# pglira/simpleICP

Measured on AMD Instinct MI355X. Metric: ICP iterations/sec (kNN correspondences/sec in `correspondences_per_s`), 10M-vs-10M pts, higher is better.
Workload: dtype f64; 1 GPU; C4 synthetic 10000000-vs-10000000 surface (SURVEY 8d generator), correspondences=1000, neighbors=10, exact 1-NN (bit-identical to brute force); n_fixed=10000000, n_movable=10000000, correspondences=1000, neighbors=10, parallelism=movable-cloud index shards x1, queries replicated

## Files before the change

simpleicp_amd/_lib.py:

```python
from __future__ import annotations

import ctypes as C
import os
from pathlib import Path

import numpy as np

PKG = Path(__file__).resolve().parent
LIB_PATH = Path(os.environ["SICP_LIBRARY"]) if os.environ.get("SICP_LIBRARY") else PKG / "libsimpleicp_hip.so"

FIX, MOV = 0, 1
OK, ERR_INVALID, ERR_HIP, ERR_NO_DEVICE, ERR_TOO_FEW, ERR_NUMERIC, ERR_EXCHANGE = 0, -1, -2, -3, -4, -5, -6
XCHG_ALLGATHER_F64, XCHG_SUM_F64, XCHG_MIN_U64, XCHG_MAX_U64 = 1, 2, 3, 4
PART_CLOUD, PART_QUERIES = 0, 1
K_KNN1, K_KNNK, K_NORMALEQ, K_SELECT, K_XCHG = 0, 1, 2, 3, 4
ABI_VERSION = 7
KERNEL_NAMES = {K_KNN1: "match", K_KNNK: "knnk_scan", K_NORMALEQ: "solve", K_SELECT: "reject_select", K_XCHG: "exchange"}
MATCH_KERNELS = {0: "k_knn1_scan", 1: "k_knn1_fscan", 2: "k_grid_nn", 3: "k_knn1_frec", 5: "k_grid_nn16", 6: "k_grid_nn16f"}

EXPORTS = [
    "sicp_abi_version", "sicp_last_error", "sicp_device_count", "sicp_ctx_create", "sicp_ctx_destroy",
    "sicp_ctx_device_name", "sicp_cloud_upload", "sicp_cloud_upload_columns", "sicp_cloud_upload_start", "sicp_cloud_upload_wait", "sicp_cloud_size", "sicp_cloud_transform",
    "sicp_cloud_download", "sicp_cloud_download_columns", "sicp_cloud_download_both", "sicp_cloud_set_planarity", "sicp_knn", "sicp_select_in_range", "sicp_estimate_normals", "sicp_icp_setup", "sicp_icp_iterate",
    "sicp_icp_run", "sicp_icp_get_state", "sicp_icp_uncertainties", "sicp_icp_normal_equations", "sicp_params_to_H",
# ... 5 lines not shown
BATCH_EXPORTS = ["sicp_batch_version", "sicp_icp_run_batch", "sicp_ctx_lean"]
BATCH_VERSION = 1
BATCH_PATH_BATCHED, BATCH_PATH_FALLBACK = 1, 2

DEVICE_EXPORTS = ["sicp_device_version", "sicp_cloud_upload_strided", "sicp_select_n_device", "sicp_select_positions",
                  "sicp_cloud_write_strided"]
DEVICE_VERSION = 1
DT_F32, DT_F64 = 1, 2

NORMALS_EXPORTS = ["sicp_normals_version", "sicp_cloud_set_normals", "sicp_normal_angle_set", "sicp_corr_reject_normal_angle",
                   "sicp_normal_angle_info", "sicp_normal_cache_read"]
NORMALS_VERSION = 1

VOXEL_EXPORTS = ["sicp_voxel_version", "sicp_voxel_select", "sicp_voxel_select_masked"]
VOXEL_VERSION = 1


class BackendError(RuntimeError):

    def __init__(self, message, code=None):
        super().__init__(message)
        self.code = code


class IterParams(C.Structure):
    _fields_ = [("x", C.c_double * 6), ("obs", C.c_double * 6), ("obs_weight", C.c_double * 6),
                ("min_planarity", C.c_double), ("distance_weight", C.c_double), ("max_lm_steps", C.c_int64)]


class IterResult(C.Structure):
# ... 104 lines not shown
        for name in DEVICE_EXPORTS:
            getattr(L, name).restype = cint
    if all(hasattr(L, name) for name in NORMALS_EXPORTS):
        L.sicp_cloud_set_normals.argtypes = [vp, cint, vp, vp, i64, i64]
        L.sicp_normal_angle_set.argtypes = [vp, dbl, cint]
        L.sicp_corr_reject_normal_angle.argtypes = [vp, dbl, cint, vp, vp, C.POINTER(i64)]
        L.sicp_normal_angle_info.argtypes = [vp, vp]
        L.sicp_normal_cache_read.argtypes = [vp, vp, vp]
        for name in NORMALS_EXPORTS:
            getattr(L, name).restype = cint
    if all(hasattr(L, name) for name in VOXEL_EXPORTS):
        L.sicp_voxel_select.argtypes = [vp, cint, vp, i64, dbl, vp, vp, C.POINTER(i64)]
        L.sicp_voxel_select_masked.argtypes = [vp, cint, vp, i64, dbl, vp, vp, C.POINTER(i64)]
        for name in VOXEL_EXPORTS:
            getattr(L, name).restype = cint
    _lib = L
    return L


def _ptr(a):
    if a is None:
        return None
    if isinstance(a, np.ndarray):
        return a.ctypes.data_as(C.c_void_p)
    if hasattr(a, "data_ptr"):
        return C.c_void_p(a.data_ptr())
    raise TypeError(f"unsupported buffer type {type(a)}")


def _f64(a):
# ... 543 lines not shown
        self._chk(self._L.sicp_match_work(self._h, _ptr(out)))
        d = C.c_uint64(0)
        self._chk(self._L.sicp_match_deferred(self._h, C.byref(d)))
        return {"candidates": int(out[0]), "rows": int(out[1]), "launches": int(out[2]), "deferred": int(d.value)}

    def tail_cycles(self):
        out = np.zeros(5)
        self._chk(self._L.sicp_tail_cycles(self._h, _ptr(out)))
        return dict(zip(("load", "select", "keep", "lm", "final"), (float(v) for v in out)))

    def tail_selection(self):
        out = np.zeros(3, np.int64)
        self._chk(self._L.sicp_tail_selection(self._h, _ptr(out)))
        return {"median_rounds": int(out[0]), "mad_rounds": int(out[1]), "window_iterations": int(out[2])}

    def exchange_info(self):
        out = np.zeros(4, np.int64)
        self._chk(self._L.sicp_exchange_info(self._h, _ptr(out)))
        return {"form": ("none", "records_allgather", "key_allreduces", "query_slices")[int(out[0])], "count": int(out[1]),
                "keys_min_q": int(out[2]), "callback_serves_u64": bool(out[3])}

    def knn_work(self):
        out = np.zeros(4, np.uint64)
        self._chk(self._L.sicp_knn_work(self._h, _ptr(out)))
        return {"candidates": int(out[0]), "sweeps": int(out[1]), "slow_queries": int(out[2]), "in_ball": int(out[3])}

    def timing(self):
        out = {}
        for k, name in KERNEL_NAMES.items():
            ms, n = C.c_double(), C.c_int64()
# ... 4 lines not shown
```

simpleicp_amd/build.py:

```python
import os
import shutil
import subprocess
import sys
from concurrent.futures import ThreadPoolExecutor
from pathlib import Path

PKG = Path(__file__).resolve().parent
CSRC = PKG / "csrc"
LIB = PKG / "libsimpleicp_hip.so"
SOURCES = [CSRC / "sicp_api.cpp", CSRC / "sicp_clouds.cpp", CSRC / "sicp_search.cpp", CSRC / "sicp_icp.cpp", CSRC / "sicp_comm.cpp", CSRC / "sicp_kernels.hip", CSRC / "sicp_grid.hip", CSRC / "sicp_gridf.hip", CSRC / "sicp_tail.hip", CSRC / "sicp_reject.hip", CSRC / "sicp_lm.hip", CSRC / "sicp_batch.hip", CSRC / "sicp_device.hip", CSRC / "sicp_nangle.hip", CSRC / "sicp_voxel.hip", CSRC / "sicp_io.cpp"]
HEADERS = [CSRC / "sicp_internal.h", CSRC / "sicp_host.h", CSRC / "sicp_lanes.h", CSRC / "sicp_solver.h", CSRC / "sicp_normals.h", CSRC / "sicp_grid_dev.h",
           CSRC / "sicp_grid_nn_one.inc", CSRC / "sicp_knn_sweep4.inc", CSRC / "sicp_tail_body.inc", PKG.parent / "include" / "simpleicp_hip.h",
           PKG.parent / "include" / "simpleicp_hip_batch.h", PKG.parent / "include" / "simpleicp_hip_device.h",
           PKG.parent / "include" / "simpleicp_hip_normals.h", PKG.parent / "include" / "simpleicp_hip_voxel.h"]
COMPILE = ["--offload-arch=gfx950", "-O3", "-std=c++17", "-ffp-contract=off", "-fPIC",
           "-fvisibility=hidden", "-Wall", "-pthread", "-mllvm", "-amdgpu-mfma-vgpr-form",
           "-mllvm", "-amdgpu-kernarg-preload-count=16"]
LINK = ["--offload-arch=gfx950", "-shared", "-fPIC", "-pthread"]
OBJ = PKG / "_obj"
LIB_ASAN = OBJ / "libsimpleicp_hip_asan.so"


def hipcc():
    exe = shutil.which("hipcc") or "/opt/rocm/bin/hipcc"
    if not Path(exe).exists():
        raise RuntimeError("hipcc not found: cannot build libsimpleicp_hip.so")
    return exe


# ... 79 lines not shown
```

simpleicp_amd/csrc/sicp_api.cpp:

```cpp
#include "sicp_host.h"

namespace sicph {

thread_local std::string g_err;

int fail(int code, const char *fmt, ...)
{
    char buf[512];
    va_list ap;
    va_start(ap, fmt);
    vsnprintf(buf, sizeof buf, fmt, ap);
    va_end(ap);
    g_err = buf;
    return code;
}

}

int sicp_io_fail(int code, const char *fmt, ...)
{
    char buf[512];
    va_list ap;
    va_start(ap, fmt);
    vsnprintf(buf, sizeof buf, fmt, ap);
// ... 120 lines not shown
    if (rc == SICP_OK && hipMemsetAsync(c->ticket.p, 0, 4 * sizeof(unsigned), c->stream) != hipSuccess) rc = SICP_ERR_HIP;
    if (rc != SICP_OK) { sicp_ctx_destroy(c); return rc; }
    if (const char *e = std::getenv("SICP_ORDER_MIN_Q")) c->order_min_q = std::atol(e);
    if (const char *e = std::getenv("SICP_KNN_SWEEP")) c->knn_sweep = std::atoi(e) != 0;
    if (const char *e = std::getenv("SICP_KNN_BATCH")) c->knn_batch = std::atol(e);
    if (const char *e = std::getenv("SICP_KNN_GROUP")) c->knn_group = std::atoi(e);
    if (const char *e = std::getenv("SICP_NN16_MIN_Q")) c->nn16_min_q = std::atol(e);
    if (const char *e = std::getenv("SICP_NN16")) c->nn16_filter = !std::strcmp(e, "exact") ? 0 : !std::strcmp(e, "far") ? 1 : 2;
    if (const char *e = std::getenv("SICP_BOXES")) { c->use_boxes = std::atoi(e) != 0; c->boxes_always = std::atoi(e) >= 2; }
    if (const char *e = std::getenv("SICP_NN16F_MIN_Q")) { c->nn16f_min_q = std::atol(e); c->nn16f_min_q_forced = true; }
    if (const char *e = std::getenv("SICP_FAR_MOVE")) { const double t = std::atof(e); if (t >= 0) c->far_move = t; }
    if (const char *e = std::getenv("SICP_COARSE_MIN_N")) c->coarse_min_n = std::atol(e);
    if (const char *e = std::getenv("SICP_LM")) c->lm_one_launch = std::strcmp(e, "launches") != 0;
    if (const char *e = std::getenv("SICP_HSEL_WINDOW")) c->hsel_window = std::atoi(e) != 0;
    if (const char *e = std::getenv("SICP_TAIL_WINDOW")) c->tail_window = std::atoi(e) != 0;
    if (const char *e = std::getenv("SICP_TEST_BARRIER_FAULT")) c->test_barrier_fault = std::atoi(e);
    if (const char *e = std::getenv("SICP_NN_GROUP")) { const int v = std::atoi(e); if (v == 8 || v == 16) c->nn_group = v; }
    if (const char *e = std::getenv("SICP_XCHG_KEYS_MIN_Q")) c->xkeys_min_q = std::atol(e);
    if (const char *e = std::getenv("SICP_COMM_TIMEOUT_S")) { const double v = std::atof(e); if (v > 0) c->xchg_timeout_s = 2.0 * v; }
    if (const char *e = std::getenv("SICP_FSCAN")) c->fscan_variant = !std::strcmp(e, "inline") ? 1 : 0;
    if (const char *e = std::getenv("SICP_FSCAN_CAP")) c->fscan_cap = std::atol(e);
    if (const char *e = std::getenv("SICP_SOLVE_TRACE")) {
        c->solve_trace = true;
        c->host_trace = std::strstr(e, "host") != nullptr;
        c->trace_sel = std::strstr(e, "sel") != nullptr; c->trace_eval = std::strstr(e, "eval") != nullptr;
    }
    if (const char *e = std::getenv("SICP_SOLVE")) c->solve_mode = !std::strcmp(e, "fused") ? 1 : !std::strcmp(e, "host") ? 2 : 0;
    if (const char *e = std::getenv("SICP_KNN1"))
        c->knn1_mode = !std::strcmp(e, "exact") ? 1 : !std::strcmp(e, "filter") ? 2 : !std::strcmp(e, "grid") ? 3 : 0;
    *ctx_out = c;
// ... 91 lines not shown
    HIPCHK(hipMemcpyAsync(out, c->match_work.p + 3, sizeof(uint64_t), hipMemcpyDeviceToHost, c->stream));
    return sync(c);
}
SICP_EXPORT int sicp_tail_cycles(sicp_ctx *c, double out5[5])
{
    if (!c || !out5) return fail(SICP_ERR_INVALID, "null argument");
    std::memcpy(out5, c->last_tail_cycles, sizeof c->last_tail_cycles);
    return SICP_OK;
}
SICP_EXPORT int sicp_tail_selection(sicp_ctx *c, int64_t out3[3])
{
    if (!c || !out3) return fail(SICP_ERR_INVALID, "null argument");
    out3[0] = c->last_sel_rounds[0]; out3[1] = c->last_sel_rounds[1]; out3[2] = c->sel_window_hits;
    return SICP_OK;
}
SICP_EXPORT int sicp_knn_work(sicp_ctx *c, uint64_t out4[4])
{
    if (!c || !out4) return fail(SICP_ERR_INVALID, "null argument");
    HIPCHK(hipSetDevice(c->device));
    HIPCHK(hipMemcpyAsync(out4, c->match_work.p + 4, 4 * sizeof(uint64_t), hipMemcpyDeviceToHost, c->stream));
    return sync(c);
}
SICP_EXPORT int sicp_timing_reset(sicp_ctx *c)
{
    if (!c) return fail(SICP_ERR_INVALID, "null ctx");
    if (!c->pending.empty()) CHK(sync(c));
    HIPCHK(hipMemsetAsync(c->match_work.p, 0, 8 * sizeof(unsigned long long), c->stream));
    for (int i = 0; i < SICP_K_COUNT; ++i) { c->t_ms[i] = 0; c->t_n[i] = 0; }
    return SICP_OK;
}
// ... 10 lines not shown
```

simpleicp_amd/csrc/sicp_batch.hip:

```cpp
#include "sicp_host.h"
#include "../../include/simpleicp_hip_batch.h"

#include <set>

namespace {

void set_status(sicp_batch_member &m, int rc)
{
    m.status = rc;
    if (rc == SICP_OK) m.error[0] = '\0';
    else std::snprintf(m.error, sizeof m.error, "%s", sicp_last_error());
}

bool batchable(sicp_ctx *c, const sicp_batch_member &m)
{
    if (check_iter_args(c, &m.params) != SICP_OK) return false;
    if (!device_tail(c) || c->Q > SOLVE_MAX_Q || !takes_grid_search(c)) return false;
    if (normal_angle_on(c)) return false;
    return !(c->timing || c->count_work || c->host_trace || c->solve_trace);
}

struct MemberRun {
    int64_t idx;
    double xcur[6];
// ... 82 lines not shown
        run.push_back(r);
    }
    const long B = (long)tab.size();
    if (B > 0) {
        std::vector<uint32_t> map;
        int depth = 1 << 30;
        int64_t max_all = 0;
        for (long k = 0; k < B; ++k) {
            const long blocks = ((long)tab[k].A.Q + 3) / 4;
            tab[k].blk0 = (uint32_t)map.size();
            map.insert(map.end(), (size_t)blocks, (uint32_t)k);
            depth = std::min(depth, mem[run[k].idx].ctx->chain_depth);
            max_all = std::max(max_all, tab[k].max_it);
        }
        const long nblk = (long)map.size();
        const int epts[4] = {1, 2, 4, 8};
        long b_off[4], b_cnt[4];
        for (int b = 0; b < 4; ++b) {
            b_off[b] = (long)map.size();
            for (long k = 0; k < B; ++k)
                if (icp_tail_ept(tab[k].A.Q) == epts[b]) map.push_back((uint32_t)k);
            b_cnt[b] = (long)map.size() - b_off[b];
        }
        for (long k = 0; k < B; ++k) tab[k].ring = c0->h_batch_ring + (size_t)k * REC_RING * REC_DOUBLES;
        const hipStream_t s0 = c0->stream;
        const int rc = [&]() -> int {
        for (long k = 0; k < B; ++k) HIPCHK(hipStreamWaitEvent(s0, mem[run[k].idx].ctx->batch_ev, 0));
        HIPCHK(hipMemcpyAsync(c0->batch_tab.p, tab.data(), (size_t)B * sizeof(BatchMember), hipMemcpyHostToDevice, s0));
        HIPCHK(hipMemcpyAsync(c0->batch_map.p, map.data(), map.size() * sizeof(uint32_t), hipMemcpyHostToDevice, s0));
        for (long k = 0; k < B; ++k) {
            sicp_ctx *c = mem[run[k].idx].ctx;
            c->have_prev_match = true;
            c->last_match_kernel = 2;
        }

        double seqs[REC_RING];
        int64_t launched = 0, completed = 0;
        auto all_over = [&]() {
            for (long k = 0; k < B; ++k) if (!run[k].over && launched < tab[k].max_it) return false;
            return true;
        };
        while (true) {
            while (launched < max_all && launched - completed < depth && !all_over()) {
                const double seq = (double)(++c0->solve_seq);
                const int slot = (int)(launched % REC_RING);
                seqs[slot] = seq;
                launch_grid_nn_batch(s0, c0->batch_tab.p, c0->batch_map.p, nblk, launched);
                for (int b = 0; b < 4; ++b)
                    if (b_cnt[b] > 0) launch_icp_tail_batch(s0, epts[b], c0->batch_tab.p, c0->batch_map.p + b_off[b], b_cnt[b], launched, slot, seq);
                HIPCHK(hipGetLastError());
                ++launched;
            }
            if (completed == launched) break;
            const int slot = (int)(completed % REC_RING);
            for (long k = 0; k < B; ++k) {
                if (completed >= tab[k].max_it) continue;
                const double *o = tab[k].ring + (size_t)slot * REC_DOUBLES;
                CHK(wait_ticket(c0, o + REC_TICKET, seqs[slot]));
                if ((int)o[REC_STATUS] == 3 || run[k].over) { run[k].over = true; continue; }
                sicp_batch_member &m = mem[run[k].idx];
                const int rc = take_record(m.ctx, &m.params, o, m.results, &m.iterations, run[k].xcur, &run[k].last_move, &run[k].over);
                if (rc != SICP_OK) set_status(m, rc);
            }
            ++completed;
// ... 19 lines not shown
```

simpleicp_amd/csrc/sicp_host.h:

```cpp
#ifndef SICP_HOST_H
#define SICP_HOST_H

#include <hip/hip_runtime.h>
#include <rccl/rccl.h>
#include <dlfcn.h>
#include <sched.h>

#include <algorithm>
#include <atomic>
#include <chrono>
#include <cmath>
#include <cstdarg>
#include <cstdio>
#include <cstdlib>
#include <cstring>
#include <limits>
#include <condition_variable>
#include <memory>
#include <mutex>
#include <string>
#include <thread>
#include <vector>

#include "../../include/simpleicp_hip.h"
// ... 194 lines not shown
    DevBuf<uint8_t> flag, keep;
    DevBuf<double> small;
    DevBuf<double> ne_partial;
    DevBuf<unsigned> ticket;
    double *h_small = nullptr;
    double *h_dl = nullptr;
    hipEvent_t dl_ev[4] = {nullptr, nullptr, nullptr, nullptr};
    bool have_iter = false;
    bool have_corr = false;
    NormalAngle na;
    DevBuf<float> corr_pl;
    double last_x[6] = {0}, last_w = 1.0, last_obs[6] = {0}, last_ow[6] = {0};
    double last_ne[30] = {0};
    double last_tail_cycles[5] = {0};
    long last_sel_rounds[2] = {0, 0}, sel_window_hits = 0;
    bool have_last_ne = false;
    int solve_mode = 0;
    bool grid_target_forced = false;
    double grid_target = 16.0;
    bool host_trace = false;
    bool solve_trace = false;
    bool trace_sel = false, trace_eval = false;
    long solve_seq = 0;
    DevBuf<IcpDev> icp_dev;
    DevBuf<LmDev> lm_dev;
    LmDev *h_lm = nullptr;
    DevBuf<double> resid2;
    int resid_slot = 0;
    int lm_evals = 4;
    double *h_rec = nullptr;
    IcpDev *h_state = nullptr;
    DevBuf<unsigned long long> lm_bar_buf;
    unsigned long long lm_bar = 0;
    bool lm_one_launch = true;
    unsigned long long hsel_bar = 0;
    int test_barrier_fault = 0;
    bool tail_window = true;
    bool reject_prior = false;
    bool hsel_window = true;
    long hsel_run_launches = 0;
    bool hsel_dirty = false;
    int nn_group = 0;
    int chain_depth = 4;
    DevBuf<BatchMember> batch_tab;
    DevBuf<uint32_t> batch_map;
    double *h_batch_ring = nullptr;
    long batch_ring_members = 0;
    hipEvent_t batch_ev = nullptr;
    DevBuf<uint32_t> sel_blk;
    DevBuf<int64_t> sel_pos;
    DevBuf<unsigned long long> vx_tab;
    DevBuf<uint32_t> vx_slot;
// ... 144 lines not shown
```

simpleicp_amd/csrc/sicp_icp.cpp:

```cpp
#include "sicp_host.h"

namespace sicph {

void euler_R(const double a[3], double R[9])
{
    const double c1 = std::cos(a[0]), s1 = std::sin(a[0]);
    const double c2 = std::cos(a[1]), s2 = std::sin(a[1]);
    const double c3 = std::cos(a[2]), s3 = std::sin(a[2]);
    R[0] = c2 * c3;                 R[1] = -c2 * s3;                R[2] = s2;
    R[3] = c1 * s3 + s1 * s2 * c3;  R[4] = c1 * c3 - s1 * s2 * s3;  R[5] = -s1 * c2;
    R[6] = s1 * s3 - c1 * s2 * c3;  R[7] = s1 * c3 + c1 * s2 * s3;  R[8] = c1 * c2;
}

void euler_dR(const double a[3], double dR[27])
{
    const double c1 = std::cos(a[0]), s1 = std::sin(a[0]);
    const double c2 = std::cos(a[1]), s2 = std::sin(a[1]);
    const double c3 = std::cos(a[2]), s3 = std::sin(a[2]);
    double *A = dR, *B = dR + 9, *C = dR + 18;
    A[0] = 0; A[1] = 0; A[2] = 0;
    A[3] = -s1 * s3 + c1 * s2 * c3;  A[4] = -s1 * c3 - c1 * s2 * s3;  A[5] = -c1 * c2;
    A[6] = c1 * s3 + s1 * s2 * c3;   A[7] = c1 * c3 - s1 * s2 * s3;   A[8] = -s1 * c2;
    B[0] = -s2 * c3;       B[1] = s2 * s3;        B[2] = c2;
    B[3] = s1 * c2 * c3;   B[4] = -s1 * c2 * s3;  B[5] = s1 * s2;
// ... 139 lines not shown
    c->resid_slot = 0; c->resid_sharded = false;
    HIPCHK(hipMemcpyAsync(c->m_idx.p, sel_idx, (size_t)Q * sizeof(int64_t), hipMemcpyDefault, c->stream));
    launch_gather_queries(c->stream, cl.x(), cl.y(), cl.z(), c->m_idx.p, Q, c->qpad, c->q.p, c->q.p + c->qpad, c->q.p + 2 * c->qpad);
    HIPCHK(hipGetLastError());
    HIPCHK(hipMemcpyAsync(c->normals.p, normals, (size_t)3 * Q * sizeof(float), hipMemcpyDefault, c->stream));
    HIPCHK(hipMemcpyAsync(c->planarity.p, planarity, (size_t)Q * sizeof(float), hipMemcpyDefault, c->stream));
    c->have_iter = false;
    c->have_corr = false;
    c->have_prev_match = false;
#ifndef SICP_TEST_REVERT_SLOT_FIX
    c->slot_cnt = -1;
#endif
    c->q_order_lo = -1; c->q_order_cnt = 0;
    c->hsel_run_launches = 0;
    c->sel_window_hits = 0; c->last_sel_rounds[0] = c->last_sel_rounds[1] = 0;
    c->last_xchg_form = 0; c->xchg_count = 0;
    c->reject_prior = false;
    c->na.counters_stale = true;
    return sync(c);
}

namespace sicph {

int too_few(long long n)
{
    return fail(SICP_ERR_TOO_FEW, "Too few correspondences! At least 6 correspondences are needed to estimate the 6 "
                                  "rigid body transformation parameters. The current number of correspondences is %lld.", n);
}

int check_iter_args(sicp_ctx *c, const sicp_iter_params *P)
// ... 24 lines not shown
    HIPCHK(hipMemcpyAsync(c->icp_dev.p, &hs, sizeof hs, hipMemcpyHostToDevice, c->stream));
    return SICP_OK;
}

TailArgs tail_args(const sicp_ctx *c, const sicp_iter_params *P0, double min_change)
{
    const Cloud &cl = c->cloud[SICP_MOV];
    TailArgs A;
    for (int j = 0; j < 6; ++j) { A.obs[j] = P0->obs[j]; A.ow[j] = P0->obs_weight[j]; }
    A.min_change = min_change;
    A.seq = 0.0;
    A.min_planarity = (float)P0->min_planarity;
    A.max_steps = P0->max_lm_steps > 0 ? (int)P0->max_lm_steps : 100;
    A.Q = (int)c->Q;
    A.window = c->tail_window ? 1 : 0;
    A.pl2 = cl.pl_n > 0 ? cl.pl.p : nullptr;
    A.pl2_n = cl.pl_n;
    return A;
}

int take_record(sicp_ctx *c, const sicp_iter_params *P0, const double *o, sicp_iter_result *results, int64_t *done_out,
                double xcur[6], double *last_move, bool *over)
{
    const long Q = c->Q;
    const Cloud &cl = c->cloud[SICP_MOV];
    const bool small_q = Q <= SOLVE_MAX_Q;
    const int status = (int)o[REC_STATUS];
    int rc = SICP_OK;
    sicp_iter_result &R = results[*done_out];
    std::memset(&R, 0, sizeof R);
// ... 15 lines not shown
        for (int j = 0; j < 3; ++j) { da += (R.x[j] - xcur[j]) * (R.x[j] - xcur[j]); dt += (R.x[3 + j] - xcur[3 + j]) * (R.x[3 + j] - xcur[3 + j]); }
        *last_move = std::sqrt(dt) + std::sqrt(da) * cl.rmax;
        c->last_move = *last_move;
    }
    std::memcpy(xcur, R.x, 6 * sizeof(double));
    c->last_w = R.weight_used;
    std::memcpy(c->last_obs, P0->obs, sizeof c->last_obs);
    std::memcpy(c->last_ow, P0->obs_weight, sizeof c->last_ow);
    std::memcpy(c->last_ne, o + 20, sizeof c->last_ne);
    c->have_last_ne = true;
    c->resid_slot = small_q ? 0 : (int)o[REC_RESID_SLOT];
    if (small_q) {
        std::memcpy(c->last_tail_cycles, o + 50, 5 * sizeof(double));
        c->last_sel_rounds[0] = (long)o[56]; c->last_sel_rounds[1] = (long)o[58];
        if (o[56] == 0.0 && o[58] == 0.0) ++c->sel_window_hits;
    }
    if (c->solve_trace && small_q)
        std::fprintf(stderr, "[tail] cycles: load+dist %.0f select %.0f (median %.0f in %.0f rounds, MAD %.0f in %.0f) keep %.0f lm %.0f "
                             "(%lld evals %.0f, %lld steps, solves %.0f, accept %.0f) final %.0f\n",
                     o[50], o[51], o[55], o[56], o[57], o[58], o[52], o[53], (long long)R.ne_evals, o[59], (long long)R.lm_steps, o[60], o[62], o[54]);
    if (c->solve_trace && small_q && c->trace_sel)
        std::fprintf(stderr, "[sel] median: atomics+barrier %.0f fold+barrier %.0f scan+pick %.0f (more rounds %.0f) gather+barrier %.0f rank %.0f | "
                             "MAD: %.0f %.0f %.0f (%.0f) %.0f %.0f\n", o[38], o[39], o[40], o[41], o[42], o[43], o[44], o[45], o[46], o[47], o[48], o[49]);
    if (c->solve_trace && small_q && c->trace_eval)
        std::fprintf(stderr, "[eval] rows + LDS writes %.0f barrier %.0f MFMA Gram %.0f block write + barrier %.0f fold %.0f\n", o[38], o[39], o[40], o[41], o[42]);
    if (o[REC_CONVERGED] != 0.0) *over = true;
    return rc;
}


// ... 635 lines not shown
```

simpleicp_amd/csrc/sicp_internal.h:

```cpp
#pragma once
#include <hip/hip_runtime.h>
#include <stdint.h>

namespace sicp {

struct Xf { double m[12]; };

constexpr int    KNN_BLOCK = 256;
constexpr int    KNN1_R    = 4;
constexpr int    TILE_PTS  = 1024;
constexpr int    FS_TILE   = 512;
constexpr int    FS_R      = 8;
constexpr int    FS_G      = 8;
constexpr int    REJECT_MAX_Q = 16384;
constexpr int    QPAD      = 2048;
constexpr int    NE_BLOCK  = 256;
constexpr int    NE_MAX_GRID = 1024;
constexpr long   STATS_MB_MIN_Q = 16384;
#define SICP_PAD_COORD 1.0e300

constexpr int SOLVE_MAX_Q = 2048;
void launch_fill_f32(hipStream_t s, float *dst, long n, float v);
void launch_corr_planarity(hipStream_t s, uint8_t *alive, const float *pl1, const float *pl2, float min_planarity, long Q);
void launch_scatter_f32(hipStream_t s, float *dst, const int64_t *rows, const float *vals, long m);
// ... 17 lines not shown
    long pl2_n;
    float min_planarity;
    double *dist;
    uint8_t *flag;
    double *pack;
    double *pack_idx;
};
struct TailArgs {
    double obs[6], ow[6];
    double min_change;
    double seq;
    float min_planarity;
    int max_steps;
    int Q;
    int window;
    const float *pl2;
    long pl2_n;
};
constexpr int REC_STATUS = 18;
constexpr int REC_CONVERGED = 19;
constexpr int REC_RESID_SLOT = 61;
constexpr int REC_TICKET = 63;
constexpr int REC_DOUBLES = 64;
void launch_icp_tail(hipStream_t s, const double *qx, const double *qy, const double *qz, const float *normals,
                     const double *p2, const TailArgs &A, IcpDev *st, const double *dist, const uint8_t *flag,
                     uint8_t *keep, double *resid, double *rec);

struct LmDev {
    double x[6], sc[6];
    double xt[6], sct[6];
    double G[2][64];
    double stat[2][2];
    double shift;
    double w, cost, lambda, dxmax;
    int cur, first, tries, steps, evals, done, pad[2];
};
// ... 32 lines not shown
    const double *qx, *qy, *qz;
    const float *normals, *planarity;
    double *m_d2; int64_t *m_idx; double *m_p2;
    double *dist; uint8_t *flag, *keep; double *resid;
    const uint32_t *cell_start; const void *rec;
    GridGeom G;
    double rmax;
    int64_t idx_base;
    const double *prev0;
    double *ring;
    TailArgs A;
    int64_t max_it;
    uint32_t blk0, pad;
};
void launch_grid_nn_batch(hipStream_t s, const BatchMember *tab, const uint32_t *blk_member, long blocks, long launch);
void launch_icp_tail_batch(hipStream_t s, int ept, const BatchMember *tab, const uint32_t *members, long count, long launch, int slot,
                           double seq);
int  icp_tail_ept(long Q);

constexpr int NN_TIGHT = 1;
constexpr int NN_APPROX = 2;
struct GridSearch {
    const double *qx = nullptr, *qy = nullptr, *qz = nullptr;
    long Q = 0;
    const uint32_t *order = nullptr;
    const double *prev_p2 = nullptr;
    const void *qrec = nullptr; void *pslot = nullptr;
    uint8_t *state = nullptr;
    GridGeom G = {}; const uint32_t *cell_start = nullptr; const void *rec = nullptr;
    const GridLevel *coarse = nullptr;
    const unsigned long long *cell_box = nullptr;
    const void *recf = nullptr; const double *c0 = nullptr; double eps_p = 0.0;
// ... 109 lines not shown
```

simpleicp_amd/csrc/sicp_lanes.h:

```cpp
#ifndef SICP_LANES_H
#define SICP_LANES_H

#include <hip/hip_runtime.h>

namespace sicp {

typedef unsigned v2u_t __attribute__((ext_vector_type(2)));

template <int CTRL>
__device__ __forceinline__ unsigned dpp_mov(unsigned v)
{
    return (unsigned)__builtin_amdgcn_update_dpp(0, (int)v, CTRL, 0xF, 0xF, true);
}

template <int J>
__device__ __forceinline__ unsigned lane_xor32(unsigned v)
{
    if constexpr (J == 1) return dpp_mov<0xB1>(v);
    else if constexpr (J == 2) return dpp_mov<0x4E>(v);
    else if constexpr (J == 4) return dpp_mov<0x1B>(dpp_mov<0x141>(v));
    else if constexpr (J == 8) return dpp_mov<0x141>(dpp_mov<0x140>(v));
    else if constexpr (J == 16) { const v2u_t r = __builtin_amdgcn_permlane16_swap(v, v, false, false); return (threadIdx.x & 16) ? r.x : r.y; }
    else { const v2u_t r = __builtin_amdgcn_permlane32_swap(v, v, false, false); return (threadIdx.x & 32) ? r.x : r.y; }
}

template <int J>
__device__ __forceinline__ unsigned long long lane_xor64(unsigned long long v)
{
    const unsigned lo = lane_xor32<J>((unsigned)v), hi = lane_xor32<J>((unsigned)(v >> 32));
    return ((unsigned long long)hi << 32) | lo;
}

template <int J>
__device__ __forceinline__ double lane_xor_f64(double v)
{
    return __longlong_as_double((long long)lane_xor64<J>((unsigned long long)__double_as_longlong(v)));
}

__device__ __forceinline__ double wsum(double v)
{
    v += lane_xor_f64<32>(v);
    v += lane_xor_f64<16>(v);
    v += lane_xor_f64<8>(v);
    v += lane_xor_f64<4>(v);
    v += lane_xor_f64<2>(v);
    v += lane_xor_f64<1>(v);
    return v;
}

__device__ __forceinline__ unsigned wscan_u32(unsigned v)
{
// ... 61 lines not shown
```

simpleicp_amd/csrc/sicp_solver.h:

```cpp
#ifndef SICP_SOLVER_H
#define SICP_SOLVER_H

#include <hip/hip_runtime.h>

#include "sicp_internal.h"

namespace sicp {
namespace {

__device__ __forceinline__ void xfm(const double (&H)[12], double x, double y, double z, double &ox, double &oy, double &oz)
{
    double t;
    t = H[0] * x;  t = fma(H[1], y, t);  t = fma(H[2], z, t);   ox = t + H[3];
    t = H[4] * x;  t = fma(H[5], y, t);  t = fma(H[6], z, t);   oy = t + H[7];
    t = H[8] * x;  t = fma(H[9], y, t);  t = fma(H[10], z, t);  oz = t + H[11];
}
__device__ __forceinline__ double pdist(double dx, double dy, double dz, float nx, float ny, float nz)
{
    const double a = dx * (double)nx, b = dy * (double)ny, c = dz * (double)nz;
    return (a + b) + c;
}
__device__ __attribute__((noinline)) double2 sincos_cold(double a)
{
    double s, c;
// ... 89 lines not shown
    for (int i = 0; i < 6; ++i) {
#pragma unroll
        for (int k = 0; k < i; ++k) b[i] = fma(-M[i][k], b[k], b[i]);
    }
#pragma unroll
    for (int i = 5; i >= 0; --i) {
        double t = b[i] * inv[i];
#pragma unroll
        for (int k = i + 1; k < 6; ++k) t = fma(-M[k][i], dx[k], t);
        dx[i] = t;
    }
    return ok;
}


}
}

#endif
```

simpleicp_amd/csrc/sicp_tail.hip:

```cpp
#include <hip/hip_runtime.h>
#include <stdint.h>

#include "sicp_internal.h"
#include "sicp_lanes.h"
#include "sicp_solver.h"

namespace sicp {

namespace {

typedef double v4d __attribute__((ext_vector_type(4)));

__device__ __forceinline__ unsigned long long okey(double v)
{
    const unsigned long long b = (unsigned long long)__double_as_longlong(v);
    return (b & 0x8000000000000000ull) ? ~b : (b | 0x8000000000000000ull);
}
__device__ __forceinline__ double oval(unsigned long long k)
{
    const unsigned long long b = (k & 0x8000000000000000ull) ? (k & 0x7fffffffffffffffull) : ~k;
    return __longlong_as_double((long long)b);
}

constexpr int TB = 256;
// ... 415 lines not shown
__device__ __forceinline__ void flush_rec(TailShared &S, double *rec, int count)
{
    const int lane = threadIdx.x;
    if (lane < count) __hip_atomic_store(rec + lane, S.out[lane], __ATOMIC_RELAXED, __HIP_MEMORY_SCOPE_SYSTEM);
}
__device__ __forceinline__ void publish(double *rec, double seq)
{
    asm volatile("s_waitcnt vmcnt(0)" ::: "memory");
    if (threadIdx.x == 0) {
        __hip_atomic_store(rec + REC_TICKET, seq, __ATOMIC_RELAXED, __HIP_MEMORY_SCOPE_SYSTEM);
    }
}

}

template <int EPT>
__global__ __launch_bounds__(TB, 1) void k_icp_tail(
    IcpDev *__restrict__ st,
    const double *__restrict__ dist ,
    const uint8_t *__restrict__ flag ,
    const double *__restrict__ p2, const double *__restrict__ qx, const double *__restrict__ qy, const double *__restrict__ qz,
    const float *__restrict__ normals, uint8_t *__restrict__ keep, double *__restrict__ resid, double *__restrict__ rec, TailArgs A)
{
    __shared__ TailShared S;
#include "sicp_tail_body.inc"
}

void launch_icp_tail(hipStream_t s, const double *qx, const double *qy, const double *qz, const float *normals,
                     const double *p2, const TailArgs &A, IcpDev *st, const double *dist, const uint8_t *flag,
                     uint8_t *keep, double *resid, double *rec)
{
    if (A.Q <= TB)
        hipLaunchKernelGGL(k_icp_tail<1>, dim3(1), dim3(TB), 0, s, st, dist, flag, p2, qx, qy, qz, normals, keep, resid, rec, A);
    else if (A.Q <= 2 * TB)
        hipLaunchKernelGGL(k_icp_tail<2>, dim3(1), dim3(TB), 0, s, st, dist, flag, p2, qx, qy, qz, normals, keep, resid, rec, A);
    else if (A.Q <= 4 * TB)
        hipLaunchKernelGGL(k_icp_tail<4>, dim3(1), dim3(TB), 0, s, st, dist, flag, p2, qx, qy, qz, normals, keep, resid, rec, A);
    else
        hipLaunchKernelGGL(k_icp_tail<8>, dim3(1), dim3(TB), 0, s, st, dist, flag, p2, qx, qy, qz, normals, keep, resid, rec, A);
}

template <int EPT>
__global__ __launch_bounds__(TB, 1) void k_icp_tail_batch(const BatchMember *__restrict__ tab, const uint32_t *__restrict__ members,
                                                          long launch, int slot, double seq)
{
    __shared__ TailShared S;
    const BatchMember &M = tab[members[blockIdx.x]];
    if (launch >= M.max_it) return;
    IcpDev *const st = M.st;
    const double *const dist = M.dist, *const p2 = M.m_p2, *const qx = M.qx, *const qy = M.qy, *const qz = M.qz;
    const uint8_t *const flag = M.flag;
    const float *const normals = M.normals;
    uint8_t *const keep = M.keep;
    double *const resid = M.resid;
    double *const rec = M.ring + (long)slot * REC_DOUBLES;
    TailArgs A = M.A;
    A.seq = seq;
#include "sicp_tail_body.inc"
}

int icp_tail_ept(long Q)
{
    return Q <= TB ? 1 : Q <= 2 * TB ? 2 : Q <= 4 * TB ? 4 : 8;
}

void launch_icp_tail_batch(hipStream_t s, int ept, const BatchMember *tab, const uint32_t *members, long count, long launch, int slot,
                           double seq)
{
    const dim3 g((unsigned)count), b(TB);
    switch (ept) {
    case 1: hipLaunchKernelGGL(k_icp_tail_batch<1>, g, b, 0, s, tab, members, launch, slot, seq); break;
    case 2: hipLaunchKernelGGL(k_icp_tail_batch<2>, g, b, 0, s, tab, members, launch, slot, seq); break;
    case 4: hipLaunchKernelGGL(k_icp_tail_batch<4>, g, b, 0, s, tab, members, launch, slot, seq); break;
    default: hipLaunchKernelGGL(k_icp_tail_batch<8>, g, b, 0, s, tab, members, launch, slot, seq); break;
    }
}

}
```

simpleicp_amd/csrc/sicp_tail_body.inc:

```
    const int tid = threadIdx.x, wid = tid >> 6;
    const int Q = A.Q;
    long long tk[6]; tk[0] = clock64();
    double d[EPT];
    uint8_t fb[EPT];
#pragma unroll
    for (int e = 0; e < EPT; ++e) {
        const int i = tid + e * TB;
        const int ic = i < Q ? i : Q - 1;
        d[e] = dist[ic]; fb[e] = flag[ic];
    }
    double x[6], sc[6];
#pragma unroll
    for (int j = 0; j < 6; ++j) { x[j] = st->x[j]; sc[j] = st->sc[j]; }
    const double w_state = st->w, prev_mean = st->prev_mean, prev_std = st->prev_std;
    const int done_iters = st->done_iters;
    const int stop = st->stop;
    const double pmed = st->sel_med, pmad = st->sel_mad;
    const int pcnt = st->sel_m;
    Corr<EPT> C;
#pragma unroll
    for (int e = 0; e < EPT; ++e) {
        const int i = tid + e * TB;
        const int ic = i < Q ? i : Q - 1;
        C.px[e] = p2[3 * ic]; C.py[e] = p2[3 * ic + 1]; C.pz[e] = p2[3 * ic + 2];
// ... 177 lines not shown
#pragma unroll
                for (int j = 0; j < 6; ++j) xmax = fmax(xmax, fabs(x[j]));
                if (dxmax <= 1e-13 * (1.0 + xmax)) break;
            }
            first = false;
            if (steps >= A.max_steps || nfree == 0) break;
        } else {
            lambda = lambda > 0 ? lambda * 10 : 1e-6;
            if (++tries >= 40) break;
        }
        bool ok = false;
        double dstep[6];
        SICP_FT(const long long ts0 = clock64(); t_acc += ts0 - te1;)
#pragma unroll 1
        for (; tries < 40; ++tries) {
            ok = lm_step(S.gf[wid][cur], w, x, lambda, A, dstep);
            dxmax = 0.0;
#pragma unroll
            for (int j = 0; j < 6; ++j) { xn[j] = x[j] + dstep[j]; dxmax = fmax(dxmax, fabs(dstep[j])); }
            ok = ok && (dxmax < __builtin_inf());
            if (ok) break;
            lambda = lambda > 0 ? lambda * 10 : 1e-6;
        }
        SICP_FT(t_step += clock64() - ts0;)
        if (!ok) break;
        double xm = 0.0;
#pragma unroll
        for (int j = 0; j < 6; ++j) xm = fmax(xm, fabs(x[j]));
        if (lambda == 0.0 && dxmax <= 1e-10 * (1.0 + xm)) break;
#pragma unroll
        for (int j = 0; j < 3; ++j) sincos_step(xn[j], dstep[j], sc[2 * j], sc[2 * j + 1], scn[2 * j], scn[2 * j + 1]);
    }
    tk[4] = clock64();

    const double *G = S.gf[wid][cur];
    const double gn = G[7 * 8 + 7];
    const double rmean = G[6 * 8 + 7] / gn;
    const double rvar = G[6 * 8 + 6] / gn - rmean * rmean;
    const double rstd = sqrt(rvar > 0.0 ? rvar : 0.0);
#pragma unroll
    for (int e = 0; e < EPT; ++e) {
        const int i = tid + e * TB;
        if (i < Q) resid[i] = rr[e];
    }
    const bool finite = cost < __builtin_inf();
    bool conv = false;
// ... 36 lines not shown
        else if (tid == 28) { u = 6; v = 6; }
        else { u = 7; v = 7; }
        S.out[20 + tid] = G[u * 8 + v];
    }
    if (tid == 0) {
        if (!need_w) {
            const double mean0 = d0s1 / d0n, var0 = d0s2 / d0n - mean0 * mean0;
            S.out[4] = mean0; S.out[5] = sqrt(var0 > 0.0 ? var0 : 0.0);
        }
        S.out[6] = w; S.out[7] = cost; S.out[8] = steps; S.out[9] = evals;
#pragma unroll
        for (int j = 0; j < 6; ++j) S.out[10 + j] = x[j];
        S.out[16] = rmean; S.out[17] = rstd;
        S.out[REC_STATUS] = finite ? 0.0 : 2.0;
        S.out[REC_CONVERGED] = conv ? 1.0 : 0.0;
        tk[5] = clock64();
        for (int k = 0; k < 5; ++k) S.out[50 + k] = (double)(tk[k + 1] - tk[k]);
        S.out[59] = (double)t_eval; S.out[60] = (double)t_step; S.out[62] = (double)t_acc;
        S.out[55] = (double)(tsel - tk[1]); S.out[56] = rounds[0]; S.out[57] = (double)(tk[2] - tsel); S.out[58] = rounds[1];
#ifdef SICP_EVAL_FINE_TRACE
        for (int i = 0; i < 5; ++i) S.out[38 + i] = (double)(S.evt[i + 1] - S.evt[i]);
#endif
#ifdef SICP_SEL_FINE_TRACE
        for (int wsel = 0; wsel < 2; ++wsel)
            for (int i = 0; i < 6; ++i) S.out[38 + 6 * wsel + i] = (double)(S.selt[wsel][i + 1] - S.selt[wsel][i]);
#endif

    }
    flush_rec(S, rec, REC_TICKET);
    publish(rec, A.seq);
// ... 1 lines not shown
```

Baseline: 50800 iterations/s.

## Distribute LM 6x6 Cholesky solve and sincos update across row lanes via DPP

Adds a row-parallel Levenberg-Marquardt step. Each lane of an 8-lane group owns one row of the 6x6 normal matrix and factorises it with DPP row broadcasts, so the scalar per-thread Cholesky is no longer repeated redundantly in every lane. The three sincos updates are also spread across lanes and broadcast back. It is enabled by default through a new template parameter and env toggle, and adds a counter to report which path ran. The cost is more kernel instantiations and a reliance on DPP broadcast correctness, including reuse of record slot 61, which is also REC_RESID_SLOT.

```diff
diff --git a/include/simpleicp_hip_tail.h b/include/simpleicp_hip_tail.h
--- /dev/null
+++ b/include/simpleicp_hip_tail.h
@@ -0,0 +1,16 @@
+#ifndef SIMPLEICP_HIP_TAIL_H
+#define SIMPLEICP_HIP_TAIL_H
+
+#include "simpleicp_hip.h"
+
+#ifdef __cplusplus
+extern "C" {
+#endif
+
+int sicp_tail_lm_path(sicp_ctx *ctx, int64_t out2[2]);
+
+#ifdef __cplusplus
+}
+#endif
+
+#endif
diff --git a/simpleicp_amd/_lib.py b/simpleicp_amd/_lib.py
--- a/simpleicp_amd/_lib.py
+++ b/simpleicp_amd/_lib.py
@@ -43,6 +43,8 @@
 
 VOXEL_EXPORTS = ["sicp_voxel_version", "sicp_voxel_select", "sicp_voxel_select_masked"]
 VOXEL_VERSION = 1
+
+TAIL_EXPORTS = ["sicp_tail_lm_path"]
 
 
 class BackendError(RuntimeError):
@@ -177,6 +179,9 @@
         L.sicp_voxel_select_masked.argtypes = [vp, cint, vp, i64, dbl, vp, vp, C.POINTER(i64)]
         for name in VOXEL_EXPORTS:
             getattr(L, name).restype = cint
+    if all(hasattr(L, name) for name in TAIL_EXPORTS):
+        L.sicp_tail_lm_path.argtypes = [vp, vp]
+        L.sicp_tail_lm_path.restype = cint
     _lib = L
     return L
 
@@ -750,6 +755,11 @@
         self._chk(self._L.sicp_tail_selection(self._h, _ptr(out)))
         return {"median_rounds": int(out[0]), "mad_rounds": int(out[1]), "window_iterations": int(out[2])}
 
+    def tail_lm_path(self):
+        out = np.zeros(2, dtype=np.int64)
+        self._chk(self._L.sicp_tail_lm_path(self._h, _ptr(out)))
+        return {"rows": int(out[0]), "in_lane": int(out[1])}
+
     def exchange_info(self):
         out = np.zeros(4, np.int64)
         self._chk(self._L.sicp_exchange_info(self._h, _ptr(out)))
diff --git a/simpleicp_amd/build.py b/simpleicp_amd/build.py
--- a/simpleicp_amd/build.py
+++ b/simpleicp_amd/build.py
@@ -12,7 +12,8 @@
 HEADERS = [CSRC / "sicp_internal.h", CSRC / "sicp_host.h", CSRC / "sicp_lanes.h", CSRC / "sicp_solver.h", CSRC / "sicp_normals.h", CSRC / "sicp_grid_dev.h",
            CSRC / "sicp_grid_nn_one.inc", CSRC / "sicp_knn_sweep4.inc", CSRC / "sicp_tail_body.inc", PKG.parent / "include" / "simpleicp_hip.h",
            PKG.parent / "include" / "simpleicp_hip_batch.h", PKG.parent / "include" / "simpleicp_hip_device.h",
-           PKG.parent / "include" / "simpleicp_hip_normals.h", PKG.parent / "include" / "simpleicp_hip_voxel.h"]
+           PKG.parent / "include" / "simpleicp_hip_normals.h", PKG.parent / "include" / "simpleicp_hip_voxel.h",
+           PKG.parent / "include" / "simpleicp_hip_tail.h"]
 COMPILE = ["--offload-arch=gfx950", "-O3", "-std=c++17", "-ffp-contract=off", "-fPIC",
            "-fvisibility=hidden", "-Wall", "-pthread", "-mllvm", "-amdgpu-mfma-vgpr-form",
            "-mllvm", "-amdgpu-kernarg-preload-count=16"]
diff --git a/simpleicp_amd/csrc/sicp_api.cpp b/simpleicp_amd/csrc/sicp_api.cpp
--- a/simpleicp_amd/csrc/sicp_api.cpp
+++ b/simpleicp_amd/csrc/sicp_api.cpp
@@ -1,4 +1,5 @@
 #include "sicp_host.h"
+#include "../../include/simpleicp_hip_tail.h"
 
 namespace sicph {
 
@@ -158,6 +159,7 @@
     if (const char *e = std::getenv("SICP_LM")) c->lm_one_launch = std::strcmp(e, "launches") != 0;
     if (const char *e = std::getenv("SICP_HSEL_WINDOW")) c->hsel_window = std::atoi(e) != 0;
     if (const char *e = std::getenv("SICP_TAIL_WINDOW")) c->tail_window = std::atoi(e) != 0;
+    if (const char *e = std::getenv("SICP_TAIL_LM_LANES")) c->tail_lm_lanes = std::atoi(e) != 0;
     if (const char *e = std::getenv("SICP_TEST_BARRIER_FAULT")) c->test_barrier_fault = std::atoi(e);
     if (const char *e = std::getenv("SICP_NN_GROUP")) { const int v = std::atoi(e); if (v == 8 || v == 16) c->nn_group = v; }
     if (const char *e = std::getenv("SICP_XCHG_KEYS_MIN_Q")) c->xkeys_min_q = std::atol(e);
@@ -279,6 +281,12 @@
     out3[0] = c->last_sel_rounds[0]; out3[1] = c->last_sel_rounds[1]; out3[2] = c->sel_window_hits;
     return SICP_OK;
 }
+SICP_EXPORT int sicp_tail_lm_path(sicp_ctx *c, int64_t out2[2])
+{
+    if (!c || !out2) return fail(SICP_ERR_INVALID, "null argument");
+    out2[0] = c->lm_path_iters[0]; out2[1] = c->lm_path_iters[1];
+    return SICP_OK;
+}
 SICP_EXPORT int sicp_knn_work(sicp_ctx *c, uint64_t out4[4])
 {
     if (!c || !out4) return fail(SICP_ERR_INVALID, "null argument");
diff --git a/simpleicp_amd/csrc/sicp_batch.hip b/simpleicp_amd/csrc/sicp_batch.hip
--- a/simpleicp_amd/csrc/sicp_batch.hip
+++ b/simpleicp_amd/csrc/sicp_batch.hip
@@ -120,12 +120,12 @@
             max_all = std::max(max_all, tab[k].max_it);
         }
         const long nblk = (long)map.size();
-        const int epts[4] = {1, 2, 4, 8};
-        long b_off[4], b_cnt[4];
-        for (int b = 0; b < 4; ++b) {
+        const int epts[8] = {1, 2, 4, 8, 1, 2, 4, 8};
+        long b_off[8], b_cnt[8];
+        for (int b = 0; b < 8; ++b) {
             b_off[b] = (long)map.size();
             for (long k = 0; k < B; ++k)
-                if (icp_tail_ept(tab[k].A.Q) == epts[b]) map.push_back((uint32_t)k);
+                if (icp_tail_ept(tab[k].A.Q) == epts[b] && (tab[k].A.lm_lanes != 0) == (b < 4)) map.push_back((uint32_t)k);
             b_cnt[b] = (long)map.size() - b_off[b];
         }
         for (long k = 0; k < B; ++k) tab[k].ring = c0->h_batch_ring + (size_t)k * REC_RING * REC_DOUBLES;
@@ -152,8 +152,8 @@
                 const int slot = (int)(launched % REC_RING);
                 seqs[slot] = seq;
                 launch_grid_nn_batch(s0, c0->batch_tab.p, c0->batch_map.p, nblk, launched);
-                for (int b = 0; b < 4; ++b)
-                    if (b_cnt[b] > 0) launch_icp_tail_batch(s0, epts[b], c0->batch_tab.p, c0->batch_map.p + b_off[b], b_cnt[b], launched, slot, seq);
+                for (int b = 0; b < 8; ++b)
+                    if (b_cnt[b] > 0) launch_icp_tail_batch(s0, epts[b], b < 4, c0->batch_tab.p, c0->batch_map.p + b_off[b], b_cnt[b], launched, slot, seq);
                 HIPCHK(hipGetLastError());
                 ++launched;
             }
diff --git a/simpleicp_amd/csrc/sicp_host.h b/simpleicp_amd/csrc/sicp_host.h
--- a/simpleicp_amd/csrc/sicp_host.h
+++ b/simpleicp_amd/csrc/sicp_host.h
@@ -232,6 +232,7 @@
     double last_ne[30] = {0};
     double last_tail_cycles[5] = {0};
     long last_sel_rounds[2] = {0, 0}, sel_window_hits = 0;
+    long lm_path_iters[2] = {0, 0};
     bool have_last_ne = false;
     int solve_mode = 0;
     bool grid_target_forced = false;
@@ -254,6 +255,7 @@
     unsigned long long hsel_bar = 0;
     int test_barrier_fault = 0;
     bool tail_window = true;
+    bool tail_lm_lanes = true;
     bool reject_prior = false;
     bool hsel_window = true;
     long hsel_run_launches = 0;
diff --git a/simpleicp_amd/csrc/sicp_icp.cpp b/simpleicp_amd/csrc/sicp_icp.cpp
--- a/simpleicp_amd/csrc/sicp_icp.cpp
+++ b/simpleicp_amd/csrc/sicp_icp.cpp
@@ -177,6 +177,7 @@
     c->q_order_lo = -1; c->q_order_cnt = 0;
     c->hsel_run_launches = 0;
     c->sel_window_hits = 0; c->last_sel_rounds[0] = c->last_sel_rounds[1] = 0;
+    c->lm_path_iters[0] = c->lm_path_iters[1] = 0;
     c->last_xchg_form = 0; c->xchg_count = 0;
     c->reject_prior = false;
     c->na.counters_stale = true;
@@ -231,6 +232,7 @@
     A.max_steps = P0->max_lm_steps > 0 ? (int)P0->max_lm_steps : 100;
     A.Q = (int)c->Q;
     A.window = c->tail_window ? 1 : 0;
+    A.lm_lanes = c->tail_lm_lanes ? 1 : 0;
     A.pl2 = cl.pl_n > 0 ? cl.pl.p : nullptr;
     A.pl2_n = cl.pl_n;
     return A;
@@ -276,6 +278,7 @@
         std::memcpy(c->last_tail_cycles, o + 50, 5 * sizeof(double));
         c->last_sel_rounds[0] = (long)o[56]; c->last_sel_rounds[1] = (long)o[58];
         if (o[56] == 0.0 && o[58] == 0.0) ++c->sel_window_hits;
+        ++c->lm_path_iters[o[REC_LM_ROWS] != 0.0 ? 0 : 1];
     }
     if (c->solve_trace && small_q)
         std::fprintf(stderr, "[tail] cycles: load+dist %.0f select %.0f (median %.0f in %.0f rounds, MAD %.0f in %.0f) keep %.0f lm %.0f "
diff --git a/simpleicp_amd/csrc/sicp_internal.h b/simpleicp_amd/csrc/sicp_internal.h
--- a/simpleicp_amd/csrc/sicp_internal.h
+++ b/simpleicp_amd/csrc/sicp_internal.h
@@ -55,12 +55,14 @@
     int max_steps;
     int Q;
     int window;
+    int lm_lanes;
     const float *pl2;
     long pl2_n;
 };
 constexpr int REC_STATUS = 18;
 constexpr int REC_CONVERGED = 19;
 constexpr int REC_RESID_SLOT = 61;
+constexpr int REC_LM_ROWS = 61;
 constexpr int REC_TICKET = 63;
 constexpr int REC_DOUBLES = 64;
 void launch_icp_tail(hipStream_t s, const double *qx, const double *qy, const double *qz, const float *normals,
@@ -123,8 +125,8 @@
     uint32_t blk0, pad;
 };
 void launch_grid_nn_batch(hipStream_t s, const BatchMember *tab, const uint32_t *blk_member, long blocks, long launch);
-void launch_icp_tail_batch(hipStream_t s, int ept, const BatchMember *tab, const uint32_t *members, long count, long launch, int slot,
-                           double seq);
+void launch_icp_tail_batch(hipStream_t s, int ept, bool rows, const BatchMember *tab, const uint32_t *members, long count, long launch,
+                           int slot, double seq);
 int  icp_tail_ept(long Q);
 
 constexpr int NN_TIGHT = 1;
diff --git a/simpleicp_amd/csrc/sicp_lanes.h b/simpleicp_amd/csrc/sicp_lanes.h
--- a/simpleicp_amd/csrc/sicp_lanes.h
+++ b/simpleicp_amd/csrc/sicp_lanes.h
@@ -35,6 +35,24 @@
 __device__ __forceinline__ double lane_xor_f64(double v)
 {
     return __longlong_as_double((long long)lane_xor64<J>((unsigned long long)__double_as_longlong(v)));
+}
+
+template <int L>
+__device__ __forceinline__ double row_bcast_f64(double v)
+{
+    static_assert(L >= 0 && L < 16, "a lane of the row");
+    return __builtin_amdgcn_update_dpp(0.0, v, 0x150 + L, 0xF, 0xF, false);
+}
+__device__ __forceinline__ double row_bcast_f64(double v, int l)
+{
+    switch (l) {
+    case 0: return row_bcast_f64<0>(v);
+    case 1: return row_bcast_f64<1>(v);
+    case 2: return row_bcast_f64<2>(v);
+    case 3: return row_bcast_f64<3>(v);
+    case 4: return row_bcast_f64<4>(v);
+    default: return row_bcast_f64<5>(v);
+    }
 }
 
 __device__ __forceinline__ double wsum(double v)
diff --git a/simpleicp_amd/csrc/sicp_solver.h b/simpleicp_amd/csrc/sicp_solver.h
--- a/simpleicp_amd/csrc/sicp_solver.h
+++ b/simpleicp_amd/csrc/sicp_solver.h
@@ -4,6 +4,7 @@
 #include <hip/hip_runtime.h>
 
 #include "sicp_internal.h"
+#include "sicp_lanes.h"
 
 namespace sicp {
 namespace {
@@ -127,6 +128,79 @@
 }
 
 
+__device__ __forceinline__ bool lm_step_rows(const double *G, double w, const double (&x)[6], double lambda, const TailArgs &A,
+                                             double (&dx)[6])
+{
+    const int r = threadIdx.x & 7;
+    const double w2 = w * w;
+    double owl = A.ow[5], obl = A.obs[5], xl = x[5];
+#pragma unroll
+    for (int j = 0; j < 5; ++j)
+    {
+        const double oj = A.ow[j], bj = A.obs[j], xj = x[j];
+        owl = r == j ? oj : owl; obl = r == j ? bj : obl; xl = r == j ? xj : xl;
+    }
+    const bool fl = !(owl < __builtin_inf()), ol = observed(owl);
+    const double2 *row = reinterpret_cast<const double2 *>(G + r * 8);
+    const double2 r01 = row[0], r23 = row[1], r45 = row[2];
+    const double g6 = G[r * 8 + 6], gd = G[r * 9];
+    double m[6] = {r01.x, r01.y, r23.x, r23.y, r45.x, r45.y};
+    double ad = w2 * gd;
+    if (ol) ad += owl * owl;
+    ad += lambda * ad;
+#pragma unroll
+    for (int j = 0; j < 6; ++j) {
+        const bool fj = !(A.ow[j] < __builtin_inf());
+        const double a = r == j ? ad : w2 * m[j];
+        m[j] = (fl || fj) ? (r == j ? 1.0 : 0.0) : a;
+    }
+    double g = w2 * g6;
+    if (ol) g += owl * owl * (xl - obl);
+    double b = fl ? 0.0 : -g;
+    bool ok = true;
+    double inv[6], z[6], u[6];
+#pragma unroll
+    for (int j = 0; j < 6; ++j) {
+        double t = m[j];
+#pragma unroll
+        for (int k = 0; k < j; ++k) t = fma(-m[k], row_bcast_f64(u[k], j), t);
+        const double d = row_bcast_f64(t, j);
+        ok = ok && (d > 0.0) && (d < __builtin_inf());
+        double y = __builtin_amdgcn_rcp(d);
+        y = fma(fma(-d, y, 1.0), y, y);
+        y = fma(fma(-d, y, 1.0), y, y);
+        inv[j] = y;
+        m[j] = t * y;
+        u[j] = m[j] * d;
+        z[j] = row_bcast_f64(b, j);
+        b = fma(-m[j], z[j], b);
+    }
+#pragma unroll
+    for (int i = 5; i >= 0; --i) {
+        double t = z[i] * inv[i];
+#pragma unroll
+        for (int k = i + 1; k < 6; ++k) t = fma(-row_bcast_f64(m[i], k), dx[k], t);
+        dx[i] = t;
+    }
+    return ok;
+}
+
+__device__ __forceinline__ void sincos_step_lanes(const double (&xn)[6], const double (&d)[6], const double (&sc)[6], double (&scn)[6])
+{
+    const int r = threadIdx.x & 15;
+    double a = xn[2], da = d[2], sa = sc[4], ca = sc[5];
+#pragma unroll
+    for (int j = 0; j < 2; ++j)
+    {
+        const double aj = xn[j], dj = d[j], sj = sc[2 * j], cj = sc[2 * j + 1];
+        a = r == j ? aj : a; da = r == j ? dj : da; sa = r == j ? sj : sa; ca = r == j ? cj : ca;
+    }
+    double sn, cn;
+    sincos_step(a, da, sa, ca, sn, cn);
+#pragma unroll
+    for (int j = 0; j < 3; ++j) { scn[2 * j] = row_bcast_f64(sn, j); scn[2 * j + 1] = row_bcast_f64(cn, j); }
+}
+
 }
 }
 
diff --git a/simpleicp_amd/csrc/sicp_tail.hip b/simpleicp_amd/csrc/sicp_tail.hip
--- a/simpleicp_amd/csrc/sicp_tail.hip
+++ b/simpleicp_amd/csrc/sicp_tail.hip
@@ -453,7 +453,7 @@
 
 }
 
-template <int EPT>
+template <int EPT, bool ROWS>
 __global__ __launch_bounds__(TB, 1) void k_icp_tail(
     IcpDev *__restrict__ st,
     const double *__restrict__ dist ,
@@ -469,17 +469,14 @@
                      const double *p2, const TailArgs &A, IcpDev *st, const double *dist, const uint8_t *flag,
                      uint8_t *keep, double *resid, double *rec)
 {
-    if (A.Q <= TB)
-        hipLaunchKernelGGL(k_icp_tail<1>, dim3(1), dim3(TB), 0, s, st, dist, flag, p2, qx, qy, qz, normals, keep, resid, rec, A);
-    else if (A.Q <= 2 * TB)
-        hipLaunchKernelGGL(k_icp_tail<2>, dim3(1), dim3(TB), 0, s, st, dist, flag, p2, qx, qy, qz, normals, keep, resid, rec, A);
-    else if (A.Q <= 4 * TB)
-        hipLaunchKernelGGL(k_icp_tail<4>, dim3(1), dim3(TB), 0, s, st, dist, flag, p2, qx, qy, qz, normals, keep, resid, rec, A);
-    else
-        hipLaunchKernelGGL(k_icp_tail<8>, dim3(1), dim3(TB), 0, s, st, dist, flag, p2, qx, qy, qz, normals, keep, resid, rec, A);
-}
-
-template <int EPT>
+#define SICP_TAIL(E, R) hipLaunchKernelGGL((k_icp_tail<E, R>), dim3(1), dim3(TB), 0, s, st, dist, flag, p2, qx, qy, qz, normals, keep, resid, rec, A)
+    const int ept = icp_tail_ept(A.Q);
+    if (A.lm_lanes) { if (ept == 1) SICP_TAIL(1, true); else if (ept == 2) SICP_TAIL(2, true); else if (ept == 4) SICP_TAIL(4, true); else SICP_TAIL(8, true); }
+    else { if (ept == 1) SICP_TAIL(1, false); else if (ept == 2) SICP_TAIL(2, false); else if (ept == 4) SICP_TAIL(4, false); else SICP_TAIL(8, false); }
+#undef SICP_TAIL
+}
+
+template <int EPT, bool ROWS>
 __global__ __launch_bounds__(TB, 1) void k_icp_tail_batch(const BatchMember *__restrict__ tab, const uint32_t *__restrict__ members,
                                                           long launch, int slot, double seq)
 {
@@ -503,16 +500,14 @@
     return Q <= TB ? 1 : Q <= 2 * TB ? 2 : Q <= 4 * TB ? 4 : 8;
 }
 
-void launch_icp_tail_batch(hipStream_t s, int ept, const BatchMember *tab, const uint32_t *members, long count, long launch, int slot,
-                           double seq)
+void launch_icp_tail_batch(hipStream_t s, int ept, bool rows, const BatchMember *tab, const uint32_t *members, long count, long launch,
+                           int slot, double seq)
 {
     const dim3 g((unsigned)count), b(TB);
-    switch (ept) {
-    case 1: hipLaunchKernelGGL(k_icp_tail_batch<1>, g, b, 0, s, tab, members, launch, slot, seq); break;
-    case 2: hipLaunchKernelGGL(k_icp_tail_batch<2>, g, b, 0, s, tab, members, launch, slot, seq); break;
-    case 4: hipLaunchKernelGGL(k_icp_tail_batch<4>, g, b, 0, s, tab, members, launch, slot, seq); break;
-    default: hipLaunchKernelGGL(k_icp_tail_batch<8>, g, b, 0, s, tab, members, launch, slot, seq); break;
-    }
-}
-
-}
+#define SICP_TAILB(E, R) hipLaunchKernelGGL((k_icp_tail_batch<E, R>), g, b, 0, s, tab, members, launch, slot, seq)
+    if (rows) { if (ept == 1) SICP_TAILB(1, true); else if (ept == 2) SICP_TAILB(2, true); else if (ept == 4) SICP_TAILB(4, true); else SICP_TAILB(8, true); }
+    else { if (ept == 1) SICP_TAILB(1, false); else if (ept == 2) SICP_TAILB(2, false); else if (ept == 4) SICP_TAILB(4, false); else SICP_TAILB(8, false); }
+#undef SICP_TAILB
+}
+
+}
diff --git a/simpleicp_amd/csrc/sicp_tail_body.inc b/simpleicp_amd/csrc/sicp_tail_body.inc
--- a/simpleicp_amd/csrc/sicp_tail_body.inc
+++ b/simpleicp_amd/csrc/sicp_tail_body.inc
@@ -215,7 +215,8 @@
         SICP_FT(const long long ts0 = clock64(); t_acc += ts0 - te1;)
 #pragma unroll 1
         for (; tries < 40; ++tries) {
-            ok = lm_step(S.gf[wid][cur], w, x, lambda, A, dstep);
+            if constexpr (ROWS) ok = lm_step_rows(S.gf[wid][cur], w, x, lambda, A, dstep);
+            else ok = lm_step(S.gf[wid][cur], w, x, lambda, A, dstep);
             dxmax = 0.0;
 #pragma unroll
             for (int j = 0; j < 6; ++j) { xn[j] = x[j] + dstep[j]; dxmax = fmax(dxmax, fabs(dstep[j])); }
@@ -229,8 +230,11 @@
 #pragma unroll
         for (int j = 0; j < 6; ++j) xm = fmax(xm, fabs(x[j]));
         if (lambda == 0.0 && dxmax <= 1e-10 * (1.0 + xm)) break;
-#pragma unroll
-        for (int j = 0; j < 3; ++j) sincos_step(xn[j], dstep[j], sc[2 * j], sc[2 * j + 1], scn[2 * j], scn[2 * j + 1]);
+        if constexpr (ROWS) sincos_step_lanes(xn, dstep, sc, scn);
+        else {
+#pragma unroll
+            for (int j = 0; j < 3; ++j) sincos_step(xn[j], dstep[j], sc[2 * j], sc[2 * j + 1], scn[2 * j], scn[2 * j + 1]);
+        }
     }
     tk[4] = clock64();
 
@@ -297,6 +301,7 @@
         S.out[16] = rmean; S.out[17] = rstd;
         S.out[REC_STATUS] = finite ? 0.0 : 2.0;
         S.out[REC_CONVERGED] = conv ? 1.0 : 0.0;
+        S.out[REC_LM_ROWS] = ROWS ? 1.0 : 0.0;
         tk[5] = clock64();
         for (int k = 0; k < 5; ++k) S.out[50 + k] = (double)(tk[k + 1] - tk[k]);
         S.out[59] = (double)t_eval; S.out[60] = (double)t_step; S.out[62] = (double)t_acc;
```

Result: no change. 51230 iterations/s (median of 2 runs) (+0.8%).
